# lks1248/SPH-EXA

Hardware: AMD Instinct MI355X
Metric: particle-updates/sec (whole node), Sedov -n 400, 1/2/4/8 MI355X + HBM roofline % (higher is better)
Workload: dtype f32 hydro / f64 coordinates (sph::SphTypes)

## Files before the change

### include/sphexa_hip.h

```cpp
#ifndef SPHEXA_HIP_H
#define SPHEXA_HIP_H

#include <stddef.h>
#include <stdint.h>

#ifdef __cplusplus
extern "C" {
#endif

#define SX_OK 0
#define SX_ERR_TRAVERSAL 1
#define SX_ERR_NOT_CONVERGED 2
#define SX_ERR_HIP 3
#define SX_ERR_ARG 4
#define SX_ERR_NOMEM 5

typedef struct sx_box
{
    double  lim[6];
    int32_t bnd[3];
} sx_box;

typedef struct sx_params
{
// ... 103 lines not shown
int   sx_memset(sx_ctx* ctx, void* dst, int value, size_t bytes);

int sx_sfc_keys(sx_ctx* ctx, const double* x, const double* y, const double* z, uint64_t* keys, size_t n,
                const sx_box* box);
int sx_sort_keys(sx_ctx* ctx, uint64_t* keys, uint32_t* order, size_t n);
int sx_gather(sx_ctx* ctx, const uint32_t* order, size_t n, const void* src, void* dst, int elemBytes);
int sx_compute_octree(sx_ctx* ctx, const uint64_t* sortedKeys, size_t n, uint32_t bucketSize, uint64_t* leaves,
                      uint32_t* counts, int32_t capacity, int32_t* numLeaves);
int sx_build_octree(sx_ctx* ctx, const uint64_t* leaves, int32_t numLeaves, const sx_octree* out);
int sx_node_centers(sx_ctx* ctx, const uint64_t* prefixes, int32_t numNodes, const sx_box* box, double* centers,
                    double* sizes);
int sx_leaf_layout(sx_ctx* ctx, const uint32_t* counts, int32_t numLeaves, uint32_t* layout);

int sx_compute_groups(sx_ctx* ctx, uint32_t first, uint32_t last, sx_groups* groups);
int sx_spatial_groups(sx_ctx* ctx, uint32_t first, uint32_t last, const double* x, const double* y, const double* z,
                      const sx_tree* tree, const sx_box* box, float tolFactor, uint32_t* groups, uint32_t cap,
                      sx_groups* out);
int sx_set_search_mode(sx_ctx* ctx, int mode);
int sx_find_neighbors(sx_ctx* ctx, const sx_fields* f, const sx_tree* tree, const sx_box* box,
                      const sx_params* p, uint32_t first, uint32_t last, int iterate_h, sx_nbstats* stats);
int sx_export_neighbors(sx_ctx* ctx, const uint32_t* nc, uint32_t first, uint32_t last, uint32_t ngmax,
                        uint32_t* neighbors);
int sx_import_neighbors(sx_ctx* ctx, uint32_t first, uint32_t last, uint32_t ngmax, const uint32_t* neighbors);

int sx_xmass(sx_ctx* ctx, const sx_groups* g, const sx_fields* f, const sx_params* p, const sx_box* box,
             const sx_tree* tree);
int sx_xmass_only(sx_ctx* ctx, const sx_groups* g, const sx_fields* f, const sx_params* p, const sx_box* box);
int sx_ve_def_gradh(sx_ctx* ctx, const sx_groups* g, const sx_fields* f, const sx_params* p, const sx_box* box);
int sx_eos(sx_ctx* ctx, uint32_t first, uint32_t last, float mui, double gamma, const double* temp, const float* m,
           const float* kx, const float* xm, const float* gradh, float* prho, float* c, float* rho, float* p);
int sx_iad_divv_curlv(sx_ctx* ctx, const sx_groups* g, const sx_fields* f, const sx_params* p, const sx_box* box);
int sx_av_switches(sx_ctx* ctx, const sx_groups* g, const sx_fields* f, const sx_params* p, const sx_box* box,
                   double minDt);
int sx_momentum_energy(sx_ctx* ctx, const sx_groups* g, float* groupDt, const sx_fields* f, const sx_params* p,
                       const sx_box* box, float* minDtCourant);
int sx_momentum_energy_avclean(sx_ctx* ctx, const sx_groups* g, float* groupDt, const sx_fields* f,
                               const sx_params* p, const sx_box* box, float* minDtCourant);
int sx_density(sx_ctx* ctx, const sx_groups* g, const sx_fields* f, const sx_params* p, const sx_box* box,
               const sx_tree* tree);
int sx_density_only(sx_ctx* ctx, const sx_groups* g, const sx_fields* f, const sx_params* p, const sx_box* box);
int sx_eos_std(sx_ctx* ctx, uint32_t first, uint32_t last, float mui, double gamma, const double* temp,
               const float* m, float* rho, float* p, float* c);
int sx_iad(sx_ctx* ctx, const sx_groups* g, const sx_fields* f, const sx_params* p, const sx_box* box);
int sx_momentum_energy_std(sx_ctx* ctx, const sx_groups* g, const sx_fields* f, const sx_params* p,
                           const sx_box* box, float* minDtCourant);

int sx_positions(sx_ctx* ctx, uint32_t first, uint32_t last, double dt, double dt_m1, const sx_fields* f,
                 double gamma, float muiConst, const sx_box* box);
int sx_nbody_positions(sx_ctx* ctx, uint32_t first, uint32_t last, double dt, double dt_m1, const sx_fields* f,
                       const sx_box* box, uint64_t* keys);
int sx_update_h(sx_ctx* ctx, uint32_t first, uint32_t last, uint32_t ng0, const uint32_t* nc, float* h);
int sx_update_h_groups(sx_ctx* ctx, const sx_groups* g, uint32_t ng0, const uint32_t* nc, float* h);

int sx_mark_ramp(sx_ctx* ctx, const sx_groups* g, const sx_fields* f, const sx_params* p, const sx_box* box,
                 float* markRamp);

#define SX_MAX_RUNGS 4
int sx_positions_rungs(sx_ctx* ctx, const sx_groups* g, float dt, const float* dt_m1, const uint8_t* rung,
                       const sx_fields* f, double gamma, double constCv, const sx_box* box);
int sx_drift_positions(sx_ctx* ctx, const sx_groups* g, float dt, float dt_back, const float* dt_m1,
                       const uint8_t* rung, const sx_fields* f, double gamma, double constCv);
int sx_group_divv_timestep(sx_ctx* ctx, float Krho, const sx_groups* g, const float* divv, float* groupDt);
int sx_group_acc_timestep(sx_ctx* ctx, float etaAcc, const sx_groups* g, const float* ax, const float* ay,
                          const float* az, float* groupDt);
int sx_store_rung(sx_ctx* ctx, const sx_groups* g, uint8_t rung, uint8_t* rungs);
int sx_max_divv(sx_ctx* ctx, uint32_t first, uint32_t last, const float* divv, float* maxDivv);
// ... 348 lines not shown
```

### sph-exa_amd/csrc/sx_capi.cpp

```cpp
#include <hip/hip_runtime.h>

#include <algorithm>
#include <cmath>
#include <cstdio>
#include <cstring>
#include <string>
#include <vector>

#include "../../include/sphexa_hip.h"
#include "sx_args.hpp"
#include "sx_comm.hpp"
#include "sx_direct.hpp"
#include "sx_gravity.hpp"
#include "sx_hydro.hpp"
#include "sx_kernel_poly.hpp"
#include "sx_map.hpp"
#include "sx_nbody.hpp"
#include "sx_observables.hpp"
#include "sx_profile.hpp"
#include "sx_fof.hpp"
#include "sx_twopoint.hpp"
#include "sx_spectrum.hpp"
#include "sx_tree.hpp"
#include "sx_timestep.hpp"
// ... 693 lines not shown
        EosArgs a{first, last, mui, gamma, temp, m, kx, xm, gradh, prho, cs, rho, pr};
        c->hydro().eos(a, c->stream);
        SX_HIP(c, hipGetLastError());
        return SX_OK;
    }

    int sx_iad_divv_curlv(sx_ctx* c, const sx_groups* g, const sx_fields* f, const sx_params* p, const sx_box* box)
    {
        sx_groups tmpView;
        if (int e = resolveView(c, g, tmpView, f->n)) return e;
        if (int e = checkList(c, g, p)) return e;
        Records r = records(c, f->n);
        packX(f->n, f->x, f->y, f->z, f->h, f->m, r.rx, c->stream);
        packV(f->n, f->vx, f->vy, f->vz, nullptr, r.rv, c->stream);
        packT(f->n, f->xm, f->kx, nullptr, nullptr, r.rt, c->stream);
        c->hydro().iadDivvCurlv(pairArgs(c, g, f, p, box, r), c->stream);
        SX_HIP(c, hipGetLastError());
        return SX_OK;
    }

    int sx_av_switches(sx_ctx* c, const sx_groups* g, const sx_fields* f, const sx_params* p, const sx_box* box,
                       double minDt)
    {
        sx_groups tmpView;
        if (int e = resolveView(c, g, tmpView, f->n)) return e;
        if (int e = checkList(c, g, p)) return e;
        Records r = records(c, f->n);
        packX(f->n, f->x, f->y, f->z, f->h, f->m, r.rx, c->stream);
        packV(f->n, f->vx, f->vy, f->vz, f->c, r.rv, c->stream);
        packT(f->n, f->xm, f->kx, nullptr, f->alpha, r.rt, c->stream);
        packC(f->n, f->c11, f->c12, f->c13, f->c22, f->c23, f->c33, f->divv, r.rc, c->stream, f->xm, f->kx);
        PairArgs a = pairArgs(c, g, f, p, box, r);
        a.dt       = minDt;
        c->hydro().avSwitches(a, c->stream);
        SX_HIP(c, hipGetLastError());
        return SX_OK;
    }

    int sx_momentum_energy(sx_ctx* c, const sx_groups* g, float* groupDt, const sx_fields* f, const sx_params* p,
                           const sx_box* box, float* minDtCourant)
    {
        return momentumEnergy(c, g, groupDt, f, p, box, minDtCourant, false);
    }

    int sx_momentum_energy_avclean(sx_ctx* c, const sx_groups* g, float* groupDt, const sx_fields* f,
                                   const sx_params* p, const sx_box* box, float* minDtCourant)
    {
        return momentumEnergy(c, g, groupDt, f, p, box, minDtCourant, true);
    }


    int sx_density(sx_ctx* c, const sx_groups* g, const sx_fields* f, const sx_params* p, const sx_box* box,
                   const sx_tree* tree)
    {
        sx_groups tmpView;
        if (int e = resolveView(c, g, tmpView, f->n, false)) return e;
        if (!f->rho) return fail(c, SX_ERR_ARG, "sx_density needs f->rho");
        int rc = findNeighborsView(c, f, tree, box, p, g->firstBody, g->lastBody, 1, nullptr);
        if (rc != SX_OK) return rc;
        return sx_density_only(c, g, f, p, box);
    }

    int sx_density_only(sx_ctx* c, const sx_groups* g, const sx_fields* f, const sx_params* p, const sx_box* box)
    {
        sx_groups tmpView;
        if (int e = resolveView(c, g, tmpView, f->n)) return e;
// ... 1114 lines not shown
```

### sph-exa_amd/csrc/sx_hydro.hpp

```cpp
#pragma once

#include "sx_device.hpp"

namespace sx
{

struct EosFuse
{
    const double* temp;
    double        cv;
    double        gamma;
    float *       prho, *c;
    const float * vx, *vy, *vz, *alpha;
    RecV*         rvOut;
    RecT*         rtOut;
};

struct PairArgs
{
    uint32_t first, last, numGroups, ngmax;
    int             localLists;
    const uint32_t* nidx;
    const uint32_t* nloc;
    const uint32_t* uni;
// ... 4 lines not shown
    const uint32_t* nc;
    const RecX*     rx;
    const RecV*     rv;
    const RecT*     rt;
    const RecC*     rc;
    const float2*   wh;
    const float2*   whd;
    DevBox          box;
    double          K;
    float *  xm, *kx, *gradh;
    float *  c11, *c12, *c13, *c22, *c23, *c33, *divv, *curlv;
    float*   alpha;
    float *  ax, *ay, *az;
    double*  du;
    float*   minDt;
    float*   blockDt;
    float*   groupDt;
    float  alphamin, alphamax, decay_constant;
    double        dt;
    const double* dtPtr;
    float  Atmin, Atmax, ramp, Kcour;
    float *dV11, *dV12, *dV13, *dV22, *dV23, *dV33;
    int    avClean;
    const RecS* rs;
    float* markRamp;
    const uint32_t* clusterList;
    uint32_t        listCount;
    const uint8_t* active;
    float* dtOut;
    RecT* rtOut;
    RecC* rcOut;
    uint32_t unionMax;
    EosFuse eos;
};

__device__ __forceinline__ void iadInvert(float t11, float t12, float t13, float t22, float t23, float t33, float hi,
                                          double K, float (&c)[6])
{
    auto getExp    = [](float v) { return v == 0.0f ? 0 : ilogbf(v); };
    int  tauExpSum = getExp(t11) + getExp(t12) + getExp(t13) + getExp(t22) + getExp(t23) + getExp(t33);
    const float nrm = ldexpf(1.0f, -tauExpSum / 6);
    t11 *= nrm, t12 *= nrm, t13 *= nrm, t22 *= nrm, t23 *= nrm, t33 *= nrm;
    const float det    = t11 * t22 * t33 + 2.0f * t12 * t23 * t13 - t11 * t23 * t23 - t22 * t13 * t13 - t33 * t12 * t12;
    const float factor = (float)((double)(nrm * (hi * hi * hi)) / ((double)det * K));
    c[0]               = (t22 * t33 - t23 * t23) * factor;
    c[1]               = (t13 * t23 - t33 * t12) * factor;
    c[2]               = (t12 * t23 - t22 * t13) * factor;
    c[3]               = (t11 * t33 - t13 * t13) * factor;
    c[4]               = (t13 * t12 - t11 * t23) * factor;
    c[5]               = (t11 * t22 - t12 * t12) * factor;
}

__device__ __forceinline__ float avEtaCrit(unsigned cnt)
{
    return (float)cbrt((double)32.0f * 3.14159265358979323846 / 3.0 / (double)(float)(cnt + 1));
}

template<bool EXACT>
__device__ __forceinline__ float avRvCorrection(float rx, float ry, float rz, float eta_ab, float eta_crit,
                                                const float (&gi)[6], const float (&gj)[6])
{
    const float dmy1 = rx * (gi[0] * rx + gi[1] * ry + gi[2] * rz) + (ry * (gi[3] * ry + gi[4] * rz) + rz * (gi[5] * rz));
    const float dmy2 = rx * (gj[0] * rx + gj[1] * ry + gj[2] * rz) + (ry * (gj[3] * ry + gj[4] * rz) + rz * (gj[5] * rz));
    float       dmy3 = 1.0f;
    if (eta_ab < eta_crit)
    {
// ... 81 lines not shown
```

### sph-exa_amd/csrc/sx_hydro_cluster.hip

```cpp
#include "sx_hydro.hpp"
#include "sx_kernel_poly.hpp"
#include "sx_pack12.hpp"
#include "sx_traverse.hpp"

namespace sx
{
namespace cluster
{

constexpr int kB = kCluster;

struct Clu
{
    uint32_t        c, gw, i, iSafe, U;
    bool            valid;
    unsigned        cnt;
    uint32_t        gBeg, gEnd;
    bool            packed;
    int             part;
    int             tid;
    const uint32_t* un;
    const uint32_t* nl;
    double          ox, oy, oz;
    bool            pbc;
// ... 364 lines not shown
                               r.m / a.rs[j].rho);
    };
    float t11 = 0, t12 = 0, t13 = 0, t22 = 0, t23 = 0, t33 = 0;
    bool  res = false;
    neighborLoop<CH, SPLIT>(
        cu, stage, [&](uint32_t p) { return sP[p]; },
        [&](const float4& q) {
            float rx = xi - q.x, ry = yi - q.y, rz = zi - q.z;
            pbcRule(cu, a.box, h2, rx, ry, rz);
            const float volj_w = q.w * kernelWt((rx * rx + ry * ry + rz * rz) * hiInv2);
            t11 += rx * rx * volj_w;
            t12 += rx * ry * volj_w;
            t13 += rx * rz * volj_w;
            t22 += ry * ry * volj_w;
            t23 += ry * rz * volj_w;
            t33 += rz * rz * volj_w;
        },
        res);
    {
        float v[6] = {t11, t12, t13, t22, t23, t33};
        combineShares<SPLIT>(cu, v, s_scr);
        t11 = v[0], t12 = v[1], t13 = v[2], t22 = v[3], t23 = v[4], t33 = v[5];
    }
    float cc[6];
    iadInvert(t11, t12, t13, t22, t23, t33, hi, a.K, cc);
    const float c11i = cc[0], c12i = cc[1], c13i = cc[2], c22i = cc[3], c23i = cc[4], c33i = cc[5];
    if (cu.valid && cu.part == 0)
    {
        const uint32_t i = cu.i;
        a.c11[i] = c11i, a.c12[i] = c12i, a.c13[i] = c13i, a.c22[i] = c22i, a.c23[i] = c23i, a.c33[i] = c33i;
    }
}

template<int CH, int SPLIT>
__global__ __launch_bounds__(kB * SPLIT) void iadDivvCurlvFusedKernel(PairArgs a)
{
    __shared__ float4 sP[CH];
    __shared__ float4 sV[CH];
    __shared__ float  s_red[kClusterWaves * SPLIT];
    static_assert(SPLIT == 1 || (6 * SPLIT * kCluster <= 4 * CH && 9 * SPLIT * kCluster <= 4 * CH),
                  "the share sums are combined in the record arrays");
    const Clu   cu  = setup<SPLIT>(a, s_red);
    const RecX  ri  = a.rx[cu.iSafe];
    const RecV  vi  = a.rv[cu.iSafe];
    const RecT  ti  = a.rt[cu.iSafe];
    const float kxi = ti.kx;
    const float xi = relc(ri.x, cu.ox, a.box, 0), yi = relc(ri.y, cu.oy, a.box, 1), zi = relc(ri.z, cu.oz, a.box, 2);
    const float hi = ri.h, hiInv = 1.0f / hi, hiInv2 = hiInv * hiInv, h2 = 2.0f * hi;
    float       t11 = 0, t12 = 0, t13 = 0, t22 = 0, t23 = 0, t33 = 0;
    float       M[3][3] = {{0, 0, 0}, {0, 0, 0}, {0, 0, 0}};
    bool        res = false;
    neighborLoop<CH, SPLIT>(
        cu,
        [&](uint32_t j, uint32_t slot) {
            const RecX r = a.rx[j];
            const RecV v = a.rv[j];
            const RecT t = a.rt[j];
            sP[slot]     = make_float4(relc(r.x, cu.ox, a.box, 0), relc(r.y, cu.oy, a.box, 1),
                                   relc(r.z, cu.oz, a.box, 2), t.xm / t.kx);
            sV[slot]     = make_float4(v.vx, v.vy, v.vz, t.xm);
        },
        [&](uint32_t p) { return Rec8{sP[p], sV[p]}; },
        [&](const Rec8& rec) {
            const float4& q  = rec.a;
            const float4& v  = rec.b;
            float         rx = xi - q.x, ry = yi - q.y, rz = zi - q.z;
            pbcRule(cu, a.box, h2, rx, ry, rz);
            const float W      = kernelWt((rx * rx + ry * ry + rz * rz) * hiInv2);
            const float rW[3] = {rx * W, ry * W, rz * W};
            const float px = rW[0] * q.w, py = rW[1] * q.w, pz = rW[2] * q.w;
            t11 = fmaf(px, rx, t11);
            t12 = fmaf(px, ry, t12);
            t13 = fmaf(px, rz, t13);
            t22 = fmaf(py, ry, t22);
            t23 = fmaf(py, rz, t23);
            t33 = fmaf(pz, rz, t33);
            const float f[3]  = {(v.x - vi.vx) * v.w, (v.y - vi.vy) * v.w, (v.z - vi.vz) * v.w};
#pragma unroll
            for (int aa = 0; aa < 3; ++aa)
#pragma unroll
                for (int b = 0; b < 3; ++b)
                    M[aa][b] = fmaf(rW[aa], f[b], M[aa][b]);
        },
        res);
    {
        float v[6] = {t11, t12, t13, t22, t23, t33};
        combineShares<SPLIT>(cu, v, reinterpret_cast<float*>(sP), 0u, true);
        t11 = v[0], t12 = v[1], t13 = v[2], t22 = v[3], t23 = v[4], t33 = v[5];
        float w[9] = {M[0][0], M[0][1], M[0][2], M[1][0], M[1][1], M[1][2], M[2][0], M[2][1], M[2][2]};
        combineShares<SPLIT>(cu, w, reinterpret_cast<float*>(sV));
#pragma unroll
        for (int k = 0; k < 9; ++k)
            M[k / 3][k % 3] = w[k];
    }
    float cc[6];
    iadInvert(t11, t12, t13, t22, t23, t33, hi, a.K, cc);
    const float c11i = cc[0], c12i = cc[1], c13i = cc[2], c22i = cc[3], c23i = cc[4], c33i = cc[5];
    float dV[3][3];
#pragma unroll
    for (int b = 0; b < 3; ++b)
    {
        dV[0][b] = -(c11i * M[0][b] + c12i * M[1][b] + c13i * M[2][b]);
        dV[1][b] = -(c12i * M[0][b] + c22i * M[1][b] + c23i * M[2][b]);
        dV[2][b] = -(c13i * M[0][b] + c23i * M[1][b] + c33i * M[2][b]);
    }
    const float dVx0 = dV[0][0], dVx1 = dV[1][0], dVx2 = dV[2][0];
    const float dVy0 = dV[0][1], dVy1 = dV[1][1], dVy2 = dV[2][1];
    const float dVz0 = dV[0][2], dVz1 = dV[1][2], dVz2 = dV[2][2];
    if (cu.valid && cu.part == 0)
    {
        const uint32_t i = cu.i;
        a.c11[i] = c11i, a.c12[i] = c12i, a.c13[i] = c13i, a.c22[i] = c22i, a.c23[i] = c23i, a.c33[i] = c33i;
        const float norm_kxi = (float)(a.K * (double)(hiInv * hiInv * hiInv) / (double)kxi);
        const float divv_i   = norm_kxi * (dVx0 + dVy1 + dVz2);
        a.divv[i]            = divv_i;
        if (a.rcOut) a.rcOut[i] = RecC{c11i, c12i, c13i, c22i, c23i, c33i, divv_i, ti.xm / ti.kx};
        if (a.curlv)
        {
            const float cv0 = dVz1 - dVy2, cv1 = dVx2 - dVz0, cv2 = dVy0 - dVx1;
            a.curlv[i]      = norm_kxi * norm3(cv0, cv1, cv2);
        }
        if (a.dV11)
        {
            a.dV11[i] = norm_kxi * dVx0;
            a.dV12[i] = norm_kxi * (dVx1 + dVy0);
            a.dV13[i] = norm_kxi * (dVx2 + dVz0);
            a.dV22[i] = norm_kxi * dVy1;
            a.dV23[i] = norm_kxi * (dVy2 + dVz1);
            a.dV33[i] = norm_kxi * dVz2;
        }
    }
}

template<int CH, int SPLIT, int UMIN = 0, int UMAX = 0>
__global__ __launch_bounds__(kB * SPLIT) void avSwitchesKernel(PairArgs a)
{
    __shared__ float4 sP[CH];
    __shared__ float4 sV[CH];
    __shared__ float  sD[CH];
    __shared__ float  s_red[kClusterWaves * SPLIT];
    if constexpr (UMIN > 0 || UMAX > 0)
    {
        const uint32_t blk = xcdBlock(blockIdx.x, gridDim.x);
        const uint32_t cc  = a.clusterList ? a.clusterList[blk] : blk;
        const uint32_t U   = listsB(a.lb, cc) ? a.lb.ucount[cc] : a.ucount[cc];
        if (U < (uint32_t)UMIN || (UMAX > 0 && U > (uint32_t)UMAX)) return;
    }
    const Clu   cu  = setup<SPLIT>(a, s_red);
    const RecX  ri  = a.rx[cu.iSafe];
    const RecV  vi  = a.rv[cu.iSafe];
    const RecC  ci6 = a.rc[cu.iSafe];
    const float xi = relc(ri.x, cu.ox, a.box, 0), yi = relc(ri.y, cu.oy, a.box, 1), zi = relc(ri.z, cu.oz, a.box, 2);
    const float hi = ri.h, ci = vi.c, hiInv = 1.0f / hi, hiInv2 = hiInv * hiInv, h2 = 2.0f * hi;
    const float hiInv3K     = (float)a.K * (hiInv * hiInv * hiInv);
    const float divv_i      = ci6.divv;
    float       vijsignal_i = 1.e-40f * ci;
    float       gx = 0, gy = 0, gz = 0;
    bool        res = false;
    auto        stage = [&](uint32_t j, uint32_t slot) {
        const RecX   r  = a.rx[j];
        const RecV   v  = a.rv[j];
        const float2 dv = *reinterpret_cast<const float2*>(&a.rc[j].divv);
        sP[slot] = make_float4(relc(r.x, cu.ox, a.box, 0), relc(r.y, cu.oy, a.box, 1), relc(r.z, cu.oz, a.box, 2),
                               dv.y);
        sV[slot] = make_float4(v.vx, v.vy, v.vz, v.c);
        sD[slot] = dv.x;
    };
    auto loadRec = [&](uint32_t p) { return Rec9{sP[p], sV[p], sD[p]}; };
    neighborLoop<CH, SPLIT>(
        cu, stage, loadRec,
        [&](const Rec9& r) {
            const float4& q  = r.a;
            const float4& v  = r.b;
            float         rx = xi - q.x, ry = yi - q.y, rz = zi - q.z;
            pbcRule(cu, a.box, h2, rx, ry, rz);
            const float r2    = rx * rx + ry * ry + rz * rz;
            const float rinv  = rsqrtf(r2);
            const float vx_ij = vi.vx - v.x, vy_ij = vi.vy - v.y, vz_ij = vi.vz - v.z;
            const float rv    = rx * vx_ij + ry * vy_ij + rz * vz_ij;
            const float vsig  = rv < 0.0f ? ci + v.w - 3.0f * rv * rinv : 0.0f;
            vijsignal_i       = fmaxf(vijsignal_i, vsig);
            const float fw = kernelWt(r2 * hiInv2) * (q.w * (divv_i - r.s));
            gx = fmaf(fw, rx, gx);
            gy = fmaf(fw, ry, gy);
            gz = fmaf(fw, rz, gz);
        },
        res);
    {
        float v[4] = {gx, gy, gz, vijsignal_i};
        combineShares<SPLIT>(cu, v, reinterpret_cast<float*>(sP), 8u, true);
        gx = v[0], gy = v[1], gz = v[2], vijsignal_i = v[3];
    }
    if (!cu.valid || cu.part != 0) return;
    {
        const float sx = gx, sy = gy, sz = gz;
        gx = -hiInv3K * (ci6.c11 * sx + ci6.c12 * sy + ci6.c13 * sz);
        gy = -hiInv3K * (ci6.c12 * sx + ci6.c22 * sy + ci6.c23 * sz);
        gz = -hiInv3K * (ci6.c13 * sx + ci6.c23 * sy + ci6.c33 * sz);
    }
    const float graddivv = norm3(gx, gy, gz);
    float       alphaloc = 0.0f;
    if (divv_i < 0.0f)
    {
        const float a_const = hi * hi * graddivv;
        alphaloc            = a.alphamax * a_const / (a_const + hi * fabsf(divv_i) + 0.05f * ci);
    }
    float alpha_i = a.rt[cu.i].alpha;
    if (alphaloc >= alpha_i) { alpha_i = alphaloc; }
    else
    {
        const float decay    = hi / (a.decay_constant * vijsignal_i);
        const float alphadot = ((alphaloc >= a.alphamin) ? (alphaloc - alpha_i) : (a.alphamin - alpha_i)) / decay;
        const double dt      = a.dtPtr ? *a.dtPtr : a.dt;
        alpha_i              = (float)((double)alpha_i + (double)alphadot * dt);
    }
    a.alpha[cu.i] = alpha_i;
    if (a.rtOut)
    {
        RecT t       = a.rt[cu.i];
        t.alpha      = alpha_i;
// ... 430 lines not shown
    }
    float dt_lane = INFINITY;
    if (cu.valid && cu.part == 0)
    {
        a.du[cu.i] = -a.K * 0.5 * (double)energy;
        a.ax[cu.i] = (float)(a.K * (double)mx);
        a.ay[cu.i] = (float)(a.K * (double)my);
        a.az[cu.i] = (float)(a.K * (double)mz);
        dt_lane    = tsKCourant(maxvsignali, hi, ci, a.Kcour);
        if (a.dtOut) a.dtOut[cu.i] = dt_lane;
    }
    const float wmin = waveMin(dt_lane);
    const int   wave = threadIdx.x >> 6;
    __syncthreads();
    if ((threadIdx.x & 63) == 0) s_red[wave] = wmin;
    __syncthreads();
    if (threadIdx.x == 0)
    {
        float m = s_red[0];
        for (int w = 1; w < kClusterWaves * SPLIT; ++w)
            m = s_red[w] < m ? s_red[w] : m;
        if (a.blockDt) a.blockDt[blockIdx.x] = m;
        else atomicMinPos(a.minDt, m);
    }
}

constexpr int kSplitXm = 2, kSplitVd = 2, kSplitIad = 2, kSplitAv = 2;
constexpr int kSplitAvLarge = 3;
constexpr int kSplitMe = 3;
constexpr int kSplitMeAvc = 2;
constexpr int kChIad = 1660;
constexpr int kChAv = 1470;
constexpr int kChXm = 2048, kChVd = 2000, kChAvLarge = 2048, kChMe = 2000, kChMeAvc = 1536;

static inline unsigned clusters(const PairArgs& a)
{
    return a.clusterList ? a.listCount : (a.numGroups + kClusterWaves - 1) / kClusterWaves;
}

void xmass(const PairArgs& a, hipStream_t s)
{
    if (a.numGroups && clusters(a)) xmassKernel<kChXm, kSplitXm><<<clusters(a), kB * kSplitXm, 0, s>>>(a);
}
void veDefGradh(const PairArgs& a, hipStream_t s)
{
    if (a.numGroups && clusters(a)) veDefGradhKernel<kChVd, kSplitVd><<<clusters(a), kB * kSplitVd, 0, s>>>(a);
}
void iadDivvCurlv(const PairArgs& a, hipStream_t s)
{
    if (a.numGroups && clusters(a)) iadDivvCurlvFusedKernel<kChIad, kSplitIad><<<clusters(a), kB * kSplitIad, 0, s>>>(a);
}
void avSwitches(const PairArgs& a, hipStream_t s)
{
    if (!a.numGroups || !clusters(a)) return;
    avSwitchesKernel<kChAv, kSplitAv, 0, kChAv><<<clusters(a), kB * kSplitAv, 0, s>>>(a);
    if (a.unionMax == 0 || a.unionMax > (uint32_t)kChAv)
        avSwitchesKernel<kChAvLarge, kSplitAvLarge, kChAv + 1, 0><<<clusters(a), kB * kSplitAvLarge, 0, s>>>(a);
}
__global__ __launch_bounds__(1024) void reduceBlockDtKernel(const float* v, uint32_t n, float* minDt)
{
    __shared__ float s_m[16];
    float            m = INFINITY;
    for (uint32_t i = threadIdx.x; i < n; i += blockDim.x)
        m = fminf(m, v[i]);
    m = waveMin(m);
    if ((threadIdx.x & 63) == 0) s_m[threadIdx.x >> 6] = m;
    __syncthreads();
    if (threadIdx.x == 0)
    {
        for (int w = 1; w < (int)(blockDim.x >> 6); ++w)
            m = fminf(m, s_m[w]);
        atomicMinPos(minDt, m);
    }
}
static void reduceBlockDt(const PairArgs& a, hipStream_t s)
{
    if (a.blockDt) reduceBlockDtKernel<<<1, 1024, 0, s>>>(a.blockDt, clusters(a), a.minDt);
}

static uint32_t momentumGrid(uint32_t numClusters)
{
    static int cus[64] = {};
    int        dev     = 0;
    (void)hipGetDevice(&dev);
    int& n = cus[dev & 63];
    if (n == 0)
    {
// ... 30 lines not shown
```

### sph-exa_amd/csrc/sx_sim.cpp

```cpp
#include "sx_sim_internal.hpp"

using namespace sx;
using namespace sx::sim;

namespace
{

DevBox toDevBox(const sx_box* b)
{
    DevBox d{};
    for (int k = 0; k < 6; ++k)
        d.lim[k] = b->lim[k];
    for (int k = 0; k < 3; ++k)
    {
        d.l[k]   = b->lim[2 * k + 1] - b->lim[2 * k];
        d.il[k]  = 1.0 / (b->lim[2 * k + 1] - b->lim[2 * k]);
        d.pbc[k] = b->bnd[k] == 1;
        d.fbc[k] = b->bnd[k] == 2;
        d.anyPbc |= d.pbc[k];
    }
    return d;
}


// ... 577 lines not shown
    SIM_HIP(T.begin(Kernel::veDefGradh, st));
    PairArgs va = pa;
    if (fused)
        va.eos = EosFuse{s->temp,  (double)idealGasCv(s->p.muiConst, s->p.gamma), s->p.gamma, s->prho, s->c,
                         s->vx,    s->vy, s->vz, s->alpha, s->rv, s->rt};
    if (int e = exchangeThen(
            s, H, {{s->xm, 4}},
            [&](size_t a, size_t b)
            {
                halo(a, b, [&](size_t u, size_t v)
                     { packT(v - u, s->xm + u, nullptr, nullptr, nullptr, s->rt + u, st); });
            },
            [&](const PairArgs& p) { H.veDefGradh(p, st); }, va, st))
        return e;
    SIM_HIP(T.end(Kernel::veDefGradh, st));
    SIM_HIP(T.stageEnd(Stage::VeDefGradh, st));
    if (!fused)
    {
        EosArgs ea{(uint32_t)s->first, (uint32_t)s->last, s->p.muiConst, s->p.gamma, s->temp, s->m, s->kx,
                   s->xm, s->gradh, s->prho, s->c, nullptr, nullptr};
        H.eos(ea, st);
    }
    SIM_HIP(T.stageEnd(Stage::EOS, st));
    auto packVT = [&](size_t a, size_t b)
    {
        halo(a, b,
             [&](size_t u, size_t v)
             {
                 packV(v - u, s->vx + u, s->vy + u, s->vz + u, s->c + u, s->rv + u, st);
                 packT(v - u, s->xm + u, s->kx + u, s->prho + u, s->alpha + u, s->rt + u, st);
             });
    };
    pa.rcOut = fused ? s->rc : nullptr;
    SIM_HIP(T.begin(Kernel::iadDivvCurlv, st));
    if (int e = exchangeThen(s, H, {{s->vx, 4}, {s->vy, 4}, {s->vz, 4}, {s->prho, 4}, {s->c, 4}, {s->kx, 4}},
                             packVT, [&](const PairArgs& p) { H.iadDivvCurlv(p, st); }, pa, st))
        return e;
    SIM_HIP(T.end(Kernel::iadDivvCurlv, st));
    SIM_HIP(maxFloat(s->divv, (uint32_t)s->first, (uint32_t)s->last, &s->sc->maxDivvU, st));
    SIM_HIP(T.stageEnd(Stage::IadDivvCurlv, st));
    SIM_HIP(T.begin(Kernel::avSwitches, st));
    if (int e = exchangeThen(
            s, H, {{s->c11, 4}, {s->c12, 4}, {s->c13, 4}, {s->c22, 4}, {s->c23, 4}, {s->c33, 4}, {s->divv, 4}},
            [&](size_t a, size_t b)
            {
                halo(a, b,
                     [&](size_t u, size_t v)
                     {
                         packC(v - u, s->c11 + u, s->c12 + u, s->c13 + u, s->c22 + u, s->c23 + u, s->c33 + u,
                               s->divv + u, s->rc + u, st, s->xm + u, s->kx + u);
                     });
            },
            [&](const PairArgs& p)
            {
                PairArgs q = p;
                q.rcOut    = nullptr;
                q.rtOut    = fused ? s->rt : nullptr;
                if (s->evStats && hipEventSynchronize(s->evStats) == hipSuccess) q.unionMax = s->statsHost[kStatMaxUnion];
                H.avSwitches(q, st);
            },
            pa, st))
        return e;
    pa.rcOut = nullptr;
    SIM_HIP(T.end(Kernel::avSwitches, st));
    SIM_HIP(T.stageEnd(Stage::AVswitches, st));
    auto packTa = [&](size_t a, size_t b)
    {
        halo(a, b, [&](size_t u, size_t v)
             { packT(v - u, s->xm + u, s->kx + u, s->prho + u, s->alpha + u, s->rt + u, st); });
    };
    auto launchMe = [&](const PairArgs& p) { H.momentumEnergy(p, st); };
    SIM_HIP(T.begin(Kernel::momentumEnergy, st));
    if (s->p.avClean)
    {
        if (int e = exchangeThen(s, H,
                                 {{s->dV[0], 4}, {s->dV[1], 4}, {s->dV[2], 4}, {s->dV[3], 4}, {s->dV[4], 4},
                                  {s->dV[5], 4}, {s->alpha, 4}},
                                 packTa, launchMe, pa, st))
            return e;
    }
    else if (int e = exchangeThen(s, H, {{s->alpha, 4}}, packTa, launchMe, pa, st)) return e;
    SIM_HIP(T.end(Kernel::momentumEnergy, st));
    SIM_HIP(T.stageEnd(Stage::MomentumEnergy, st));
    return SX_OK;
}

int integrateStage(sx_sim* s, StepCtx& c)
{
    hipStream_t st = c.st;
    if (int e = globalTimestep(s, c.dist, st)) return e;
    PosArgs qa = posArgs((uint32_t)s->first, (uint32_t)s->last, simFields(s), s->dbox, s->p.muiConst, s->p.gamma);
// ... 709 lines not shown
```

### sph-exa_amd/python/sphexa_amd/__init__.py

```python
import ctypes as C
import os
import re

import numpy as np

HERE = os.path.dirname(os.path.abspath(__file__))
PKG = os.path.dirname(os.path.dirname(HERE))
ROOT = os.path.dirname(PKG)
LIB_PATH = os.environ.get("SPHEXA_AMD_LIB") or os.path.join(PKG, "lib", "libsphexa_hip.so")
HEADER = os.path.join(ROOT, "include", "sphexa_hip.h")

SX_OK, SX_ERR_TRAVERSAL, SX_ERR_NOT_CONVERGED, SX_ERR_HIP, SX_ERR_ARG, SX_ERR_NOMEM = range(6)
KTABLE = 20000
GROUP = 64


class SxBox(C.Structure):
    _fields_ = [("lim", C.c_double * 6), ("bnd", C.c_int32 * 3)]


class SxParams(C.Structure):
    _fields_ = [("K", C.c_double), ("ng0", C.c_uint32), ("ngmax", C.c_uint32), ("Kcour", C.c_double),
                ("Krho", C.c_double), ("gamma", C.c_double), ("muiConst", C.c_float), ("alphamin", C.c_float),
                ("alphamax", C.c_float), ("decay_constant", C.c_float), ("Atmin", C.c_float),
# ... 535 lines not shown
        "sx_node_centers": (C.c_int, [vp, vp, i32, C.POINTER(SxBox), vp, vp]),
        "sx_leaf_layout": (C.c_int, [vp, vp, i32, vp]),
        "sx_compute_groups": (C.c_int, [vp, u32, u32, C.POINTER(SxGroups)]),
        "sx_set_search_mode": (C.c_int, [vp, C.c_int]),
        "sx_mark_ramp": (C.c_int, [vp, C.POINTER(SxGroups), C.POINTER(SxFields), C.POINTER(SxParams),
                                   C.POINTER(SxBox), vp]),
        "sx_positions_rungs": (C.c_int, [vp, C.POINTER(SxGroups), C.c_float, vp, vp, C.POINTER(SxFields), C.c_double,
                                         C.c_double, C.POINTER(SxBox)]),
        "sx_drift_positions": (C.c_int, [vp, C.POINTER(SxGroups), C.c_float, C.c_float, vp, vp, C.POINTER(SxFields),
                                         C.c_double, C.c_double]),
        "sx_group_divv_timestep": (C.c_int, [vp, C.c_float, C.POINTER(SxGroups), vp, vp]),
        "sx_group_acc_timestep": (C.c_int, [vp, C.c_float, C.POINTER(SxGroups), vp, vp, vp, vp]),
        "sx_store_rung": (C.c_int, [vp, C.POINTER(SxGroups), C.c_uint8, vp]),
        "sx_rung_timestep": (C.c_int, [vp, vp, vp, u32, C.c_float, vp, C.POINTER(SxTimestep)]),
        "sx_minimum_group_dt": (C.c_int, [vp, C.POINTER(SxTimestep), vp, vp, u32, vp, C.POINTER(C.c_float), vp]),
        "sx_extract_groups": (C.c_int, [vp, C.POINTER(SxGroups), vp, u32, u32, vp, vp]),
        "sx_spatial_groups": (C.c_int, [vp, u32, u32, vp, vp, vp, C.POINTER(SxTree), C.POINTER(SxBox), C.c_float,
                                        vp, u32, C.POINTER(SxGroups)]),
        "sx_find_neighbors": (C.c_int, [vp, C.POINTER(SxFields), C.POINTER(SxTree), C.POINTER(SxBox),
                                        C.POINTER(SxParams), u32, u32, C.c_int, C.POINTER(SxNbStats)]),
        "sx_export_neighbors": (C.c_int, [vp, vp, u32, u32, u32, vp]),
        "sx_import_neighbors": (C.c_int, [vp, u32, u32, u32, vp]),
        "sx_xmass": (C.c_int, [vp, C.POINTER(SxGroups), C.POINTER(SxFields), C.POINTER(SxParams), C.POINTER(SxBox),
                               C.POINTER(SxTree)]),
        "sx_xmass_only": (C.c_int, [vp, C.POINTER(SxGroups), C.POINTER(SxFields), C.POINTER(SxParams),
                                    C.POINTER(SxBox)]),
        "sx_ve_def_gradh": (C.c_int, [vp, C.POINTER(SxGroups), C.POINTER(SxFields), C.POINTER(SxParams),
                                      C.POINTER(SxBox)]),
        "sx_eos": (C.c_int, [vp, u32, u32, C.c_float, C.c_double, vp, vp, vp, vp, vp, vp, vp, vp, vp]),
        "sx_iad_divv_curlv": (C.c_int, [vp, C.POINTER(SxGroups), C.POINTER(SxFields), C.POINTER(SxParams),
                                        C.POINTER(SxBox)]),
        "sx_av_switches": (C.c_int, [vp, C.POINTER(SxGroups), C.POINTER(SxFields), C.POINTER(SxParams),
                                     C.POINTER(SxBox), C.c_double]),
        "sx_momentum_energy": (C.c_int, [vp, C.POINTER(SxGroups), vp, C.POINTER(SxFields), C.POINTER(SxParams),
                                         C.POINTER(SxBox), C.POINTER(C.c_float)]),
        "sx_momentum_energy_avclean": (C.c_int, [vp, C.POINTER(SxGroups), vp, C.POINTER(SxFields),
                                                 C.POINTER(SxParams), C.POINTER(SxBox), C.POINTER(C.c_float)]),
        "sx_density": (C.c_int, [vp, C.POINTER(SxGroups), C.POINTER(SxFields), C.POINTER(SxParams),
                                 C.POINTER(SxBox), C.POINTER(SxTree)]),
        "sx_density_only": (C.c_int, [vp, C.POINTER(SxGroups), C.POINTER(SxFields), C.POINTER(SxParams),
                                      C.POINTER(SxBox)]),
        "sx_eos_std": (C.c_int, [vp, u32, u32, C.c_float, C.c_double, vp, vp, vp, vp, vp]),
        "sx_iad": (C.c_int, [vp, C.POINTER(SxGroups), C.POINTER(SxFields), C.POINTER(SxParams), C.POINTER(SxBox)]),
        "sx_momentum_energy_std": (C.c_int, [vp, C.POINTER(SxGroups), C.POINTER(SxFields), C.POINTER(SxParams),
                                             C.POINTER(SxBox), C.POINTER(C.c_float)]),
        "sx_positions": (C.c_int, [vp, u32, u32, C.c_double, C.c_double, C.POINTER(SxFields), C.c_double,
                                   C.c_float, C.POINTER(SxBox)]),
        "sx_nbody_positions": (C.c_int, [vp, u32, u32, C.c_double, C.c_double, C.POINTER(SxFields), C.POINTER(SxBox),
                                         vp]),
        "sx_update_h": (C.c_int, [vp, u32, u32, u32, vp, vp]),
        "sx_update_h_groups": (C.c_int, [vp, vp, u32, vp, vp]),
        "sx_max_divv": (C.c_int, [vp, u32, u32, vp, C.POINTER(C.c_float)]),
        "sx_sim_create": (C.c_int, [C.POINTER(vp), vp, sz, C.POINTER(SxParams), C.POINTER(SxBox), u32]),
        "sx_sim_destroy": (None, [vp]),
        "sx_sim_init_sedov": (C.c_int, [vp, u32]),
        "sx_sim_set_state": (C.c_int, [vp, sz] + [vp] * 15 + [C.c_double, C.c_double]),
        "sx_sim_fields": (C.c_int, [vp, C.POINTER(SxFields), C.POINTER(vp)]),
        "sx_sim_size": (sz, [vp]),
        "sx_sim_step": (C.c_int, [vp]),
        "sx_sim_scalars": (C.c_int, [vp, C.POINTER(C.c_double)]),
        "sx_sim_stage_times": (C.c_int, [vp, C.POINTER(C.c_float), C.c_int, C.POINTER(C.c_char_p)]),
        "sx_sim_last_stats": (C.c_int, [vp, C.POINTER(SxNbStats)]),
        "sx_sim_kernel_times": (C.c_int, [vp, C.POINTER(C.c_float), C.c_int, C.POINTER(C.c_char_p)]),
        "sx_sim_set_comm": (C.c_int, [vp, vp]),
        "sx_sim_gravity_stats": (C.c_int, [vp, C.POINTER(C.c_uint64)]),
        "sx_sim_gravity_interactions": (C.c_int, [vp, C.POINTER(C.c_uint64)]),
# ... 1193 lines not shown
```

Measured before the change: 1.166 billion.

## Compute AV signal velocity in IAD kernel; lighten AV switches kernel

Moves the signal-velocity max reduction from the AV-switches pass into the fused IAD/divv/curlv kernel, which already stages neighbor velocities, and stores it per particle. The AV-switches kernel then gets a LIGHT variant that no longer loads neighbor velocity records, which cuts its memory traffic and shared-memory footprint and allows a larger chunk in one launch. In exchange the IAD kernel carries an extra shared array and reduction slot, now needs a two-launch small/large split, and a new vsig buffer is written and read back. A C API entry point is added for the fused path.

```diff
diff --git a/include/sphexa_hip.h b/include/sphexa_hip.h
--- a/include/sphexa_hip.h
+++ b/include/sphexa_hip.h
@@ -159,6 +159,8 @@
 int sx_iad_divv_curlv(sx_ctx* ctx, const sx_groups* g, const sx_fields* f, const sx_params* p, const sx_box* box);
 int sx_av_switches(sx_ctx* ctx, const sx_groups* g, const sx_fields* f, const sx_params* p, const sx_box* box,
                    double minDt);
+int sx_iad_av_fused(sx_ctx* ctx, const sx_groups* g, const sx_fields* f, const sx_params* p, const sx_box* box,
+                    double minDt);
 int sx_momentum_energy(sx_ctx* ctx, const sx_groups* g, float* groupDt, const sx_fields* f, const sx_params* p,
                        const sx_box* box, float* minDtCourant);
 int sx_momentum_energy_avclean(sx_ctx* ctx, const sx_groups* g, float* groupDt, const sx_fields* f,
diff --git a/sph-exa_amd/csrc/sx_capi.cpp b/sph-exa_amd/csrc/sx_capi.cpp
--- a/sph-exa_amd/csrc/sx_capi.cpp
+++ b/sph-exa_amd/csrc/sx_capi.cpp
@@ -749,6 +749,33 @@
         packC(f->n, f->c11, f->c12, f->c13, f->c22, f->c23, f->c33, f->divv, r.rc, c->stream, f->xm, f->kx);
         PairArgs a = pairArgs(c, g, f, p, box, r);
         a.dt       = minDt;
+        c->hydro().avSwitches(a, c->stream);
+        SX_HIP(c, hipGetLastError());
+        return SX_OK;
+    }
+
+    int sx_iad_av_fused(sx_ctx* c, const sx_groups* g, const sx_fields* f, const sx_params* p, const sx_box* box,
+                        double minDt)
+    {
+        if (!g) return fail(c, SX_ERR_ARG, "null group view");
+        if (g->groupStart && g->numGroups)
+            return fail(c, SX_ERR_ARG, "sx_iad_av_fused: explicit-group views take sx_iad_divv_curlv + sx_av_switches");
+        c->viewActive = nullptr;
+        if (int e = checkList(c, g, p)) return e;
+        if (g->firstBody >= g->lastBody) return SX_OK;
+        Records r = records(c, f->n);
+        float*  vsig = c->arena.get<float>("pair.vsig", f->n);
+        if (!r.rx || !vsig) return fail(c, SX_ERR_NOMEM, "record allocation failed");
+        packX(f->n, f->x, f->y, f->z, f->h, f->m, r.rx, c->stream);
+        packV(f->n, f->vx, f->vy, f->vz, f->c, r.rv, c->stream);
+        packT(f->n, f->xm, f->kx, nullptr, f->alpha, r.rt, c->stream);
+        PairArgs a = pairArgs(c, g, f, p, box, r);
+        if (!c->hydro().clusterLists || !a.localLists)
+            return fail(c, SX_ERR_ARG, "sx_iad_av_fused needs the fast variant's cluster lists");
+        a.vsig = vsig;
+        a.dt   = minDt;
+        c->hydro().iadDivvCurlv(a, c->stream);
+        packC(f->n, f->c11, f->c12, f->c13, f->c22, f->c23, f->c33, f->divv, r.rc, c->stream, f->xm, f->kx);
         c->hydro().avSwitches(a, c->stream);
         SX_HIP(c, hipGetLastError());
         return SX_OK;
diff --git a/sph-exa_amd/csrc/sx_hydro.hpp b/sph-exa_amd/csrc/sx_hydro.hpp
--- a/sph-exa_amd/csrc/sx_hydro.hpp
+++ b/sph-exa_amd/csrc/sx_hydro.hpp
@@ -60,6 +60,7 @@
     RecC* rcOut;
     uint32_t unionMax;
     EosFuse eos;
+    float* vsig;
 };
 
 __device__ __forceinline__ void iadInvert(float t11, float t12, float t13, float t22, float t23, float t33, float hi,
diff --git a/sph-exa_amd/csrc/sx_hydro_cluster.hip b/sph-exa_amd/csrc/sx_hydro_cluster.hip
--- a/sph-exa_amd/csrc/sx_hydro_cluster.hip
+++ b/sph-exa_amd/csrc/sx_hydro_cluster.hip
@@ -420,14 +420,39 @@
     }
 }
 
-template<int CH, int SPLIT>
+__device__ __forceinline__ float avSignalTerm(float rx, float ry, float rz, float vx_ij, float vy_ij, float vz_ij,
+                                              float ci, float cj)
+{
+    const float r2   = fmaf(rz, rz, fmaf(rx, rx, ry * ry));
+    const float rv   = fmaf(rz, vz_ij, fmaf(rx, vx_ij, ry * vy_ij));
+    const float rinv = rsqrtf(r2);
+    return rv < 0.0f ? fmaf(-3.0f * rv, rinv, ci + cj) : 0.0f;
+}
+__device__ __forceinline__ float avSignalInit(float ci) { return 1.e-40f * ci; }
+
+template<int UMIN, int UMAX>
+__device__ __forceinline__ bool otherLaunch(const PairArgs& a)
+{
+    if constexpr (UMIN > 0 || UMAX > 0)
+    {
+        const uint32_t blk = xcdBlock(blockIdx.x, gridDim.x);
+        const uint32_t cc  = a.clusterList ? a.clusterList[blk] : blk;
+        const uint32_t U   = listsB(a.lb, cc) ? a.lb.ucount[cc] : a.ucount[cc];
+        return U < (uint32_t)UMIN || (UMAX > 0 && U > (uint32_t)UMAX);
+    }
+    return false;
+}
+
+template<int CH, int SPLIT, bool VS = false, int UMIN = 0, int UMAX = 0>
 __global__ __launch_bounds__(kB * SPLIT) void iadDivvCurlvFusedKernel(PairArgs a)
 {
     __shared__ float4 sP[CH];
     __shared__ float4 sV[CH];
+    __shared__ float  sC[VS ? CH : 1];
     __shared__ float  s_red[kClusterWaves * SPLIT];
-    static_assert(SPLIT == 1 || (6 * SPLIT * kCluster <= 4 * CH && 9 * SPLIT * kCluster <= 4 * CH),
+    static_assert(SPLIT == 1 || (6 * SPLIT * kCluster <= 4 * CH && (VS ? 10 : 9) * SPLIT * kCluster <= 4 * CH),
                   "the share sums are combined in the record arrays");
+    if (otherLaunch<UMIN, UMAX>(a)) return;
     const Clu   cu  = setup<SPLIT>(a, s_red);
     const RecX  ri  = a.rx[cu.iSafe];
     const RecV  vi  = a.rv[cu.iSafe];
@@ -437,19 +462,24 @@
     const float hi = ri.h, hiInv = 1.0f / hi, hiInv2 = hiInv * hiInv, h2 = 2.0f * hi;
     float       t11 = 0, t12 = 0, t13 = 0, t22 = 0, t23 = 0, t33 = 0;
     float       M[3][3] = {{0, 0, 0}, {0, 0, 0}, {0, 0, 0}};
+    float       vijsignal_i = avSignalInit(vi.c);
     bool        res = false;
-    neighborLoop<CH, SPLIT>(
-        cu,
-        [&](uint32_t j, uint32_t slot) {
-            const RecX r = a.rx[j];
-            const RecV v = a.rv[j];
-            const RecT t = a.rt[j];
-            sP[slot]     = make_float4(relc(r.x, cu.ox, a.box, 0), relc(r.y, cu.oy, a.box, 1),
-                                   relc(r.z, cu.oz, a.box, 2), t.xm / t.kx);
-            sV[slot]     = make_float4(v.vx, v.vy, v.vz, t.xm);
-        },
-        [&](uint32_t p) { return Rec8{sP[p], sV[p]}; },
-        [&](const Rec8& rec) {
+    auto        stage = [&](uint32_t j, uint32_t slot) {
+        const RecX r = a.rx[j];
+        const RecV v = a.rv[j];
+        const RecT t = a.rt[j];
+        sP[slot]     = make_float4(relc(r.x, cu.ox, a.box, 0), relc(r.y, cu.oy, a.box, 1), relc(r.z, cu.oz, a.box, 2),
+                                   t.xm / t.kx);
+        sV[slot]     = make_float4(v.vx, v.vy, v.vz, t.xm);
+        if constexpr (VS) sC[slot] = v.c;
+    };
+    auto loadRec = [&](uint32_t p) {
+        if constexpr (VS) return Rec9{sP[p], sV[p], sC[p]};
+        else return Rec8{sP[p], sV[p]};
+    };
+    neighborLoop<CH, SPLIT, !VS>(
+        cu, stage, loadRec,
+        [&](const auto& rec) {
             const float4& q  = rec.a;
             const float4& v  = rec.b;
             float         rx = xi - q.x, ry = yi - q.y, rz = zi - q.z;
@@ -469,14 +499,19 @@
 #pragma unroll
                 for (int b = 0; b < 3; ++b)
                     M[aa][b] = fmaf(rW[aa], f[b], M[aa][b]);
+            if constexpr (VS)
+                vijsignal_i = fmaxf(vijsignal_i, avSignalTerm(rx, ry, rz, -(v.x - vi.vx), -(v.y - vi.vy),
+                                                              -(v.z - vi.vz), vi.c, rec.s));
         },
         res);
     {
         float v[6] = {t11, t12, t13, t22, t23, t33};
         combineShares<SPLIT>(cu, v, reinterpret_cast<float*>(sP), 0u, true);
         t11 = v[0], t12 = v[1], t13 = v[2], t22 = v[3], t23 = v[4], t33 = v[5];
-        float w[9] = {M[0][0], M[0][1], M[0][2], M[1][0], M[1][1], M[1][2], M[2][0], M[2][1], M[2][2]};
-        combineShares<SPLIT>(cu, w, reinterpret_cast<float*>(sV));
+        float w[VS ? 10 : 9] = {M[0][0], M[0][1], M[0][2], M[1][0], M[1][1], M[1][2], M[2][0], M[2][1], M[2][2]};
+        if constexpr (VS) w[9] = vijsignal_i;
+        combineShares<SPLIT>(cu, w, reinterpret_cast<float*>(sV), VS ? 512u : 0u);
+        if constexpr (VS) vijsignal_i = w[9];
 #pragma unroll
         for (int k = 0; k < 9; ++k)
             M[k / 3][k % 3] = w[k];
@@ -502,6 +537,7 @@
         const float norm_kxi = (float)(a.K * (double)(hiInv * hiInv * hiInv) / (double)kxi);
         const float divv_i   = norm_kxi * (dVx0 + dVy1 + dVz2);
         a.divv[i]            = divv_i;
+        if constexpr (VS) a.vsig[i] = vijsignal_i;
         if (a.rcOut) a.rcOut[i] = RecC{c11i, c12i, c13i, c22i, c23i, c33i, divv_i, ti.xm / ti.kx};
         if (a.curlv)
         {
@@ -520,20 +556,15 @@
     }
 }
 
-template<int CH, int SPLIT, int UMIN = 0, int UMAX = 0>
+template<int CH, int SPLIT, int UMIN = 0, int UMAX = 0, bool LIGHT = false>
 __global__ __launch_bounds__(kB * SPLIT) void avSwitchesKernel(PairArgs a)
 {
     __shared__ float4 sP[CH];
-    __shared__ float4 sV[CH];
+    __shared__ float4 sV[LIGHT ? 1 : CH];
     __shared__ float  sD[CH];
     __shared__ float  s_red[kClusterWaves * SPLIT];
-    if constexpr (UMIN > 0 || UMAX > 0)
-    {
-        const uint32_t blk = xcdBlock(blockIdx.x, gridDim.x);
-        const uint32_t cc  = a.clusterList ? a.clusterList[blk] : blk;
-        const uint32_t U   = listsB(a.lb, cc) ? a.lb.ucount[cc] : a.ucount[cc];
-        if (U < (uint32_t)UMIN || (UMAX > 0 && U > (uint32_t)UMAX)) return;
-    }
+    static_assert(SPLIT == 1 || 4 * SPLIT * kCluster <= 4 * CH, "the share sums are combined in the record array");
+    if (otherLaunch<UMIN, UMAX>(a)) return;
     const Clu   cu  = setup<SPLIT>(a, s_red);
     const RecX  ri  = a.rx[cu.iSafe];
     const RecV  vi  = a.rv[cu.iSafe];
@@ -542,38 +573,51 @@
     const float hi = ri.h, ci = vi.c, hiInv = 1.0f / hi, hiInv2 = hiInv * hiInv, h2 = 2.0f * hi;
     const float hiInv3K     = (float)a.K * (hiInv * hiInv * hiInv);
     const float divv_i      = ci6.divv;
-    float       vijsignal_i = 1.e-40f * ci;
+    float       vijsignal_i = avSignalInit(ci);
     float       gx = 0, gy = 0, gz = 0;
     bool        res = false;
     auto        stage = [&](uint32_t j, uint32_t slot) {
         const RecX   r  = a.rx[j];
-        const RecV   v  = a.rv[j];
         const float2 dv = *reinterpret_cast<const float2*>(&a.rc[j].divv);
         sP[slot] = make_float4(relc(r.x, cu.ox, a.box, 0), relc(r.y, cu.oy, a.box, 1), relc(r.z, cu.oz, a.box, 2),
                                dv.y);
-        sV[slot] = make_float4(v.vx, v.vy, v.vz, v.c);
+        if constexpr (!LIGHT)
+        {
+            const RecV v = a.rv[j];
+            sV[slot]     = make_float4(v.vx, v.vy, v.vz, v.c);
+        }
         sD[slot] = dv.x;
     };
-    auto loadRec = [&](uint32_t p) { return Rec9{sP[p], sV[p], sD[p]}; };
+    auto loadRec = [&](uint32_t p) {
+        if constexpr (LIGHT) return Rec5{sP[p], sD[p]};
+        else return Rec9{sP[p], sV[p], sD[p]};
+    };
     neighborLoop<CH, SPLIT>(
         cu, stage, loadRec,
-        [&](const Rec9& r) {
+        [&](const auto& r) {
             const float4& q  = r.a;
-            const float4& v  = r.b;
             float         rx = xi - q.x, ry = yi - q.y, rz = zi - q.z;
             pbcRule(cu, a.box, h2, rx, ry, rz);
-            const float r2    = rx * rx + ry * ry + rz * rz;
-            const float rinv  = rsqrtf(r2);
-            const float vx_ij = vi.vx - v.x, vy_ij = vi.vy - v.y, vz_ij = vi.vz - v.z;
-            const float rv    = rx * vx_ij + ry * vy_ij + rz * vz_ij;
-            const float vsig  = rv < 0.0f ? ci + v.w - 3.0f * rv * rinv : 0.0f;
-            vijsignal_i       = fmaxf(vijsignal_i, vsig);
+            const float r2 = rx * rx + ry * ry + rz * rz;
+            if constexpr (!LIGHT)
+            {
+                const float4& v = r.b;
+                vijsignal_i = fmaxf(vijsignal_i, avSignalTerm(rx, ry, rz, vi.vx - v.x, vi.vy - v.y, vi.vz - v.z, ci, v.w));
+            }
             const float fw = kernelWt(r2 * hiInv2) * (q.w * (divv_i - r.s));
             gx = fmaf(fw, rx, gx);
             gy = fmaf(fw, ry, gy);
             gz = fmaf(fw, rz, gz);
         },
         res);
+    if constexpr (LIGHT)
+    {
+        float v[3] = {gx, gy, gz};
+        combineShares<SPLIT>(cu, v, reinterpret_cast<float*>(sP), 0u, true);
+        gx = v[0], gy = v[1], gz = v[2];
+        vijsignal_i = a.vsig[cu.iSafe];
+    }
+    else
     {
         float v[4] = {gx, gy, gz, vijsignal_i};
         combineShares<SPLIT>(cu, v, reinterpret_cast<float*>(sP), 8u, true);
@@ -1070,6 +1114,7 @@
 constexpr int kChIad = 1660;
 constexpr int kChAv = 1470;
 constexpr int kChXm = 2048, kChVd = 2000, kChAvLarge = 2048, kChMe = 2000, kChMeAvc = 1536;
+constexpr int kChIadVs = 1470, kChIadVsLarge = 2048, kSplitIadVsLarge = 3, kChAvLight = 2040;
 
 static inline unsigned clusters(const PairArgs& a)
 {
@@ -1086,11 +1131,25 @@
 }
 void iadDivvCurlv(const PairArgs& a, hipStream_t s)
 {
-    if (a.numGroups && clusters(a)) iadDivvCurlvFusedKernel<kChIad, kSplitIad><<<clusters(a), kB * kSplitIad, 0, s>>>(a);
+    if (!a.numGroups || !clusters(a)) return;
+    if (!a.vsig)
+    {
+        iadDivvCurlvFusedKernel<kChIad, kSplitIad><<<clusters(a), kB * kSplitIad, 0, s>>>(a);
+        return;
+    }
+    iadDivvCurlvFusedKernel<kChIadVs, kSplitIad, true, 0, kChIadVs><<<clusters(a), kB * kSplitIad, 0, s>>>(a);
+    if (a.unionMax == 0 || a.unionMax > (uint32_t)kChIadVs)
+        iadDivvCurlvFusedKernel<kChIadVsLarge, kSplitIadVsLarge, true, kChIadVs + 1, 0>
+            <<<clusters(a), kB * kSplitIadVsLarge, 0, s>>>(a);
 }
 void avSwitches(const PairArgs& a, hipStream_t s)
 {
     if (!a.numGroups || !clusters(a)) return;
+    if (a.vsig)
+    {
+        avSwitchesKernel<kChAvLight, kSplitAv, 0, 0, true><<<clusters(a), kB * kSplitAv, 0, s>>>(a);
+        return;
+    }
     avSwitchesKernel<kChAv, kSplitAv, 0, kChAv><<<clusters(a), kB * kSplitAv, 0, s>>>(a);
     if (a.unionMax == 0 || a.unionMax > (uint32_t)kChAv)
         avSwitchesKernel<kChAvLarge, kSplitAvLarge, kChAv + 1, 0><<<clusters(a), kB * kSplitAvLarge, 0, s>>>(a);
diff --git a/sph-exa_amd/csrc/sx_sim.cpp b/sph-exa_amd/csrc/sx_sim.cpp
--- a/sph-exa_amd/csrc/sx_sim.cpp
+++ b/sph-exa_amd/csrc/sx_sim.cpp
@@ -633,9 +633,23 @@
              });
     };
     pa.rcOut = fused ? s->rc : nullptr;
+    if (fused)
+    {
+        pa.vsig = s->mem.get<float>("pair.vsig", s->cap);
+        if (!pa.vsig) return SX_ERR_NOMEM;
+    }
+    auto unionMax = [&]() -> uint32_t
+    { return s->evStats && hipEventSynchronize(s->evStats) == hipSuccess ? s->statsHost[kStatMaxUnion] : 0u; };
     SIM_HIP(T.begin(Kernel::iadDivvCurlv, st));
-    if (int e = exchangeThen(s, H, {{s->vx, 4}, {s->vy, 4}, {s->vz, 4}, {s->prho, 4}, {s->c, 4}, {s->kx, 4}},
-                             packVT, [&](const PairArgs& p) { H.iadDivvCurlv(p, st); }, pa, st))
+    if (int e = exchangeThen(
+            s, H, {{s->vx, 4}, {s->vy, 4}, {s->vz, 4}, {s->prho, 4}, {s->c, 4}, {s->kx, 4}}, packVT,
+            [&](const PairArgs& p)
+            {
+                PairArgs q = p;
+                if (q.vsig) q.unionMax = unionMax();
+                H.iadDivvCurlv(q, st);
+            },
+            pa, st))
         return e;
     SIM_HIP(T.end(Kernel::iadDivvCurlv, st));
     SIM_HIP(maxFloat(s->divv, (uint32_t)s->first, (uint32_t)s->last, &s->sc->maxDivvU, st));
@@ -657,7 +671,7 @@
                 PairArgs q = p;
                 q.rcOut    = nullptr;
                 q.rtOut    = fused ? s->rt : nullptr;
-                if (s->evStats && hipEventSynchronize(s->evStats) == hipSuccess) q.unionMax = s->statsHost[kStatMaxUnion];
+                if (!q.vsig) q.unionMax = unionMax();
                 H.avSwitches(q, st);
             },
             pa, st))
diff --git a/sph-exa_amd/python/sphexa_amd/__init__.py b/sph-exa_amd/python/sphexa_amd/__init__.py
--- a/sph-exa_amd/python/sphexa_amd/__init__.py
+++ b/sph-exa_amd/python/sphexa_amd/__init__.py
@@ -591,6 +591,8 @@
                                         C.POINTER(SxBox)]),
         "sx_av_switches": (C.c_int, [vp, C.POINTER(SxGroups), C.POINTER(SxFields), C.POINTER(SxParams),
                                      C.POINTER(SxBox), C.c_double]),
+        "sx_iad_av_fused": (C.c_int, [vp, C.POINTER(SxGroups), C.POINTER(SxFields), C.POINTER(SxParams),
+                                      C.POINTER(SxBox), C.c_double]),
         "sx_momentum_energy": (C.c_int, [vp, C.POINTER(SxGroups), vp, C.POINTER(SxFields), C.POINTER(SxParams),
                                          C.POINTER(SxBox), C.POINTER(C.c_float)]),
         "sx_momentum_energy_avclean": (C.c_int, [vp, C.POINTER(SxGroups), vp, C.POINTER(SxFields),
```

After: 1.120 billion. 0.96x the previous value.
